# CPCLAB-UNIPI/MPC-code

Measured on AMD Instinct MI355X. Metric: closed-loop MPC steps/sec over batch, LMPC-CSTR N=50, higher is better.
Workload: dtype f64

## Files before the change

mpc-code_amd/csrc/mpc_wave.hpp:

```cpp
#pragma once
#include "mpc_device.hpp"
#include "mpc_tp.hpp"

namespace mpc {

#ifdef MPC_WV_GENERIC_TILES
constexpr bool kWvGenericTiles = true;
#else
constexpr bool kWvGenericTiles = false;
#endif

template <int NS, int NU, int NC, int NI_>
struct WvCfg {
    static constexpr int NI = NI_;
    static constexpr int NV = NS + NU, NKF = NU * NS, NLI = NU * (NU + 1) / 2;
    static constexpr int RA = 0, RA_SZ = (NC > NKF + NLI ? NC : NKF + NLI);
    static constexpr int RG = RA_SZ, RK = RG + NV, RZ = RK + NU, ROWS = RZ + 1;
    __host__ __device__ static constexpr int ld(int N) { return (N + 1) | 1; }
    static constexpr int GUARD = 8;
    __host__ __device__ static constexpr int t_doubles(int N) { return GUARD + ROWS * NI * ld(N); }
    static constexpr int RL_A = ROWS, RL_B = RL_A + NS * NS, RL_C = RL_B + NS * NU, ROWS_LTV = RL_C + NS;
    __host__ __device__ static constexpr int t_doubles_ltv(int N) { return GUARD + ROWS_LTV * NI * ld(N); }
    static constexpr int QZN = 5 * NS + 2 * NU + 1;
    static constexpr int QN = QZN + NS;
    static constexpr int ROWS_WS = NU + 2 * NC;
    static constexpr int OUT = NU + NS + 1;
    __host__ __device__ static constexpr size_t lds_doubles(int keep_per_inst, int N) { return (size_t)t_doubles(N) + NI * QN + NI * OUT + NI * keep_per_inst; }
};

template <int NS, int NU, int NC>
struct WvIter { double sl[NC], sh[NC], ll[NC], lh[NC], u[NU], z[NS]; };

struct AReg2 { int lo, hi; };
__device__ __forceinline__ void a_put(AReg2 &r, double v)
{
    union { double d; int i[2]; } u; u.d = v;
    asm("v_accvgpr_write_b32 %0, %1" : "=a"(r.lo) : "v"(u.i[0]));
    asm("v_accvgpr_write_b32 %0, %1" : "=a"(r.hi) : "v"(u.i[1]));
}
__device__ __forceinline__ double a_get(const AReg2 &r)
{
    union { double d; int i[2]; } u;
    asm("v_accvgpr_read_b32 %0, %1" : "=v"(u.i[0]) : "a"(r.lo));
    asm("v_accvgpr_read_b32 %0, %1" : "=v"(u.i[1]) : "a"(r.hi));
    return u.d;
}
template <int NS, int NU, int NC>
struct WvIterA {
    AReg2 sl[NC], sh[NC], ll[NC], lh[NC], u[NU], z[NS];
    __device__ __forceinline__ void get(WvIter<NS, NU, NC> &X) const
    {
        MPC_UNROLL for (int i = 0; i < NC; i++) { X.sl[i] = a_get(sl[i]); X.sh[i] = a_get(sh[i]); X.ll[i] = a_get(ll[i]); X.lh[i] = a_get(lh[i]); }
        MPC_UNROLL for (int i = 0; i < NU; i++) X.u[i] = a_get(u[i]);
        MPC_UNROLL for (int i = 0; i < NS; i++) X.z[i] = a_get(z[i]);
    }
    __device__ __forceinline__ void put(const WvIter<NS, NU, NC> &X)
    {
        MPC_UNROLL for (int i = 0; i < NC; i++) { a_put(sl[i], X.sl[i]); a_put(sh[i], X.sh[i]); a_put(ll[i], X.ll[i]); a_put(lh[i], X.lh[i]); }
        MPC_UNROLL for (int i = 0; i < NU; i++) a_put(u[i], X.u[i]);
        MPC_UNROLL for (int i = 0; i < NS; i++) a_put(z[i], X.z[i]);
    }
};

struct WvInst { double mu, mu_sum, sm, inv_ncon, gscale, res_s, res_p; int stall, iters, status; bool on, warm, keep_u; };

enum : int { kWvOk0 = 1, kWvWarm = 2, kWvValid = 4, kWvKeepU = 8, kWvNoShift = 16 };

__device__ __forceinline__ double row16_sum(double v)
{
    v += dpp_move<0xB1, 0xF>(0.0, v);
    v += dpp_move<0x4E, 0xF>(0.0, v);
    v += dpp_move<0x141, 0xF>(0.0, v);
    v += dpp_move<0x140, 0xF>(0.0, v);
    return v;
}
__device__ __forceinline__ double row16_max(double v)
{
    v = dmax(v, dpp_move<0xB1, 0xF>(v, v));
    v = dmax(v, dpp_move<0x4E, 0xF>(v, v));
    v = dmax(v, dpp_move<0x141, 0xF>(v, v));
    v = dmax(v, dpp_move<0x140, 0xF>(v, v));
    return v;
}

template <int NS, int NU, bool HASM, int NC, bool MASKED, int NI, class PT, bool LTV = false, bool PAIR = false, bool RES_P = false>
__device__ __forceinline__ void wv_solve(const PT &P, double *T, const double *q, const int *iflag,
                                         WvIterA<NS, NU, NC> (&X)[PAIR ? NI / 2 : NI], WvInst (&S)[PAIR ? NI / 2 : NI], int max_iter)
{
    static_assert(!LTV || (NS <= 4 && !HASM), "time-varying stage matrices: one 4 x 4 tile per state matrix, no cross term");
    using Cfg = WvCfg<NS, NU, NC, NI>;
    using Iter = WvIter<NS, NU, NC>;
    constexpr int NV = Cfg::NV, NKF = Cfg::NKF, NLI = Cfg::NLI, RA = Cfg::RA, RG = Cfg::RG, RK = Cfg::RK;
    static_assert(NS <= 8 && NU <= 2 && NI >= 1 && NI <= 4, "stage state <= 8 (2 x 2 tiles of 4 x 4), nu <= 2 (closed-form inverse of Lambda); at most four instances per product");
    static_assert(!PAIR || NI % 2 == 0, "pairs of instances");
    constexpr int NJ = PAIR ? NI / 2 : NI;
    const int lane = threadIdx.x, N = P.N, LD = Cfg::ld(N);
    const int k = PAIR ? (lane & 31) : lane;
    const int hsel = PAIR ? (lane >> 5) : 0;
    auto ji = [&](int j) -> int { return PAIR ? 2 * j + hsel : j; };
    const bool blk_on = k < N, last = k == N - 1;
    auto tk = [&](int row, int j) -> double & { return T[(row * NI + ji(j)) * LD + k]; };
    auto un = [](double v) -> double { return PAIR ? v : uni(v); };
    auto rsum = [](double v) -> double { return PAIR ? half_sum(v) : wave_sum(v); };
    auto rmax = [](double v) -> double { return PAIR ? half_max(v) : wave_max(v); };
    MPC_STAMP_INIT

    auto launder = [](const PT &Pin) -> const PT & { const PT *pp = &Pin; asm volatile("" : "+s"(pp)); return *pp; };
    struct Bnd { double lo[NC], hi[NC]; bool fl[NC], fh[NC]; };
    auto bounds = [&](const PT &Pl, int j, Bnd &Bd) {
        const double *qd = q + ji(j) * Cfg::QN;
        MPC_UNROLL for (int i = 0; i < NC; i++) {
// ... 137 lines not shown
                const bool f_lo = fin(ulo), f_hi = fin(uhi);
                double v;
                if (Sj.warm) {
                    const double t = wave_dn1(Xj.u[i], Xj.u[i]);
                    v = (rep || Sj.keep_u) ? Xj.u[i] : t;
                    if (f_lo) v = dmax(v, ulo);
                    if (f_hi) v = dmin(v, uhi);
                } else {
                    const double us = qd[5 * NS + NU + i];
                    double push;
                    if (f_lo && f_hi) push = 0.1 * (uhi - ulo);
                    else push = 0.1 * dmax(1.0, fabs(f_lo ? ulo : (f_hi ? uhi : 0.0)));
                    v = us;
                    if (f_lo) v = dmax(v, ulo + push);
                    if (f_hi) v = dmin(v, uhi - push);
                }
                Xj.u[i] = v;
            }
            MPC_UNROLL for (int i = 0; i < NC; i++) {
                if (Sj.warm) {
                    const double tl = wave_dn1(Xj.ll[i], Xj.ll[i]), th = wave_dn1(Xj.lh[i], Xj.lh[i]);
                    ll0[i] = rep ? Xj.ll[i] : tl; lh0[i] = rep ? Xj.lh[i] : th;
                } else { ll0[i] = 0.0; lh0[i] = 0.0; }
            }
            if (LTV) {
                double Ak[NS][NS], bk[NS], xk[NS];
                MPC_UNROLL for (int i = 0; i < NS; i++) {
                    double a = blk_on ? tk(Cfg::RL_C + i, j) : 0.0;
                    MPC_UNROLL for (int l = 0; l < NU; l++) a += (blk_on ? tk(Cfg::RL_B + i * NU + l, j) : 0.0) * Xj.u[l];
                    bk[i] = a;
                    MPC_UNROLL for (int l = 0; l < NS; l++) Ak[i][l] = blk_on ? tk(Cfg::RL_A + i * NS + l, j) : 0.0;
                }
                MPC_UNROLL for (int i = 0; i < NS; i++) { double a = bk[i]; MPC_UNROLL for (int l = 0; l < NS; l++) a += Ak[i][l] * qd[l]; xk[i] = k == 0 ? a : 0.0; }
                double x00[NS];
                MPC_UNROLL for (int i = 0; i < NS; i++) x00[i] = xk[i];
                if (k == 0 || !blk_on) { MPC_UNROLL for (int i = 0; i < NS; i++) { bk[i] = x00[i]; MPC_UNROLL for (int l = 0; l < NS; l++) Ak[i][l] = 0.0; } }
                for (int s = 1; s < N; s++) {
                    double t[NS];
                    MPC_UNROLL for (int i = 0; i < NS; i++) { const double v = wave_up1(xk[i], xk[i]); t[i] = (PAIR && (k == 0 || !blk_on)) ? 0.0 : v; }
                    MPC_UNROLL for (int i = 0; i < NS; i++) { double a = bk[i]; MPC_UNROLL for (int l = 0; l < NS; l++) a += Ak[i][l] * t[l]; xk[i] = a; }
                }
                MPC_UNROLL for (int i = 0; i < NS; i++) Xj.z[i] = xk[i];
            } else {
                double xk[NS];
                MPC_UNROLL for (int i = 0; i < NS; i++) {
                    double a = qd[2 * NS + i];
                    MPC_UNROLL for (int l = 0; l < NU; l++) a += Pl.B[i][l] * Xj.u[l];
                    if (k == 0) { MPC_UNROLL for (int l = 0; l < NS; l++) a += Pl.A[i][l] * qd[l]; }
                    xk[i] = blk_on ? a : 0.0;
                }
                MPC_UNROLL for (int e = 0; e < 6; e++) {
                    const int d = 1 << e;
                    if (d < N) {
                        double t[NS];
                        MPC_UNROLL for (int i = 0; i < NS; i++) { const double v = e == 0 ? wave_up1(xk[i], xk[i]) : __shfl_up(xk[i], d, 64); t[i] = k >= d ? v : 0.0; }
                        MPC_UNROLL for (int i = 0; i < NS; i++) { double a = xk[i]; MPC_UNROLL for (int l = 0; l < NS; l++) a += Pl.Apow[e][i][l] * t[l]; xk[i] = a; }
                    }
                }
                MPC_UNROLL for (int i = 0; i < NS; i++) Xj.z[i] = xk[i];
            }
            Bnd Bd; bounds(Pl, j, Bd);
            const double ws_delta = un(qd[5 * NS + 2 * NU]);
            const double ws_smin = dmin(dmax(kWsKappa * ws_delta, kWsSMinLo), kWsSMinHi), ws_mu = kWsMuFactor * ws_smin * ws_smin;
            const double smin = Sj.warm ? ws_smin : kSMin;
            MPC_UNROLL for (int i = 0; i < NC; i++) {
                const double v = i < NU ? Xj.u[i < NU ? i : 0] : Xj.z[i >= NU ? i - NU : 0];
                Xj.sl[i] = Bd.fl[i] ? dmax(v - Bd.lo[i], smin) : 1.0; Xj.sh[i] = Bd.fh[i] ? dmax(Bd.hi[i] - v, smin) : 1.0;
                const double isl = frcp(Xj.sl[i]), ish = frcp(Xj.sh[i]);
                const double llo = Sj.warm ? dmax(ll0[i], ws_mu * isl) : kMu0 * isl, lhi = Sj.warm ? dmax(lh0[i], ws_mu * ish) : kMu0 * ish;
                Xj.ll[i] = Bd.fl[i] ? llo : 0.0; Xj.lh[i] = Bd.fh[i] ? lhi : 0.0;
            }
            X[j].put(Xj);
            phase_a(Pl, j, Sj, Xj, 0);
        }
        __builtin_amdgcn_sched_barrier(0);
    }

    MPC_TSTAMP(1);
    auto mm = [](double a, double b, double c) { return __builtin_amdgcn_mfma_f64_4x4x4f64(a, b, c, 0, 0, 0); };
    constexpr int RZ = Cfg::RZ;
    constexpr int SB = (NS + 3) / 4;
    constexpr bool VF = SB == 1 && !HASM && !kWvGenericTiles;
#define MPC_MM "v_mfma_f64_4x4x4_4b_f64 "
    struct TileCtx {
        int tr, tc; bool live;
        double *Tt, *trash;
        double Ar[SB][SB], Atr[SB][SB], Br[SB], Btr[SB];
        double *p_hu, *p_hz[SB], *p_kf, *p_k[SB], *p_kt[SB], *p_li;
        const double *p_a, *p_at, *p_b, *p_bt;
    };
    auto tile_ctx = [&](const PT &Pl) {
        int lo = threadIdx.x;
        asm volatile("" : "+v"(lo));
        TileCtx c;
        c.tr = lo >> 4; c.tc = lo & 3;
        const int tbq = (lo >> 2) & 3;
        c.live = tbq < NI;
        const int tb = c.live ? tbq : 0;
        const int tr = c.tr, tc = c.tc;
        c.Tt = T + tb * LD; c.trash = T - Cfg::GUARD;
        auto trow = [&](int row) -> double * { return c.Tt + (c.live ? row : RZ) * (NI * LD); };
        MPC_UNROLL for (int i = 0; i < SB; i++) {
            const int ri = 4 * i + tr, ci = 4 * i + tc;
            MPC_UNROLL for (int j = 0; j < SB; j++) {
                const int cj = 4 * j + tc, rj = 4 * j + tr;
                c.Ar[i][j] = (ri < NS && cj < NS) ? Pl.A[ri < NS ? ri : 0][cj < NS ? cj : 0] : 0.0;
                c.Atr[i][j] = (ri < NS && cj < NS) ? Pl.A[cj < NS ? cj : 0][ri < NS ? ri : 0] : 0.0;
                (void)rj;
            }
            c.Br[i] = (ri < NS && tc < NU) ? Pl.B[ri < NS ? ri : 0][tc < NU ? tc : 0] : 0.0;
            c.Btr[i] = (tr < NU && ci < NS) ? Pl.B[ci < NS ? ci : 0][tr < NU ? tr : 0] : 0.0;
            c.p_hz[i] = trow(ri < NS ? RG + NU + ri : RZ);
            c.p_k[i] = trow((tr < NU && ci < NS) ? RA + tr * NS + ci : RZ);
            c.p_kt[i] = trow((ri < NS && tc < NU) ? RA + tc * NS + ri : RZ);
        }
        c.p_hu = trow(tr < NU ? RG + tr : RZ); c.p_kf = trow(tr < NU ? RK + tr : RZ);
        if (LTV) {
            c.p_a = trow((tr < NS && tc < NS) ? Cfg::RL_A + tr * NS + tc : RZ); c.p_at = trow((tr < NS && tc < NS) ? Cfg::RL_A + tc * NS + tr : RZ);
            c.p_b = trow((tr < NS && tc < NU) ? Cfg::RL_B + tr * NU + tc : RZ); c.p_bt = trow((tr < NU && tc < NS) ? Cfg::RL_B + tc * NU + tr : RZ);
        }
        const int li_i = tr > tc ? tr : tc, li_j = tr > tc ? tc : tr;
        c.p_li = trow((tr < NU && tc < NU) ? RA + NKF + li_i * (li_i + 1) / 2 + li_j : RZ);
        return c;
    };
    double pd_min = 1.0;
    constexpr int PD = SB == 1 ? 4 : 2;

    auto tile_factor = [&]() {
        const PT &Pl = launder(P);
        const TileCtx c = tile_ctx(Pl);
        const int tr = c.tr, tc = c.tc; const bool live = c.live;
        double *const trash = c.trash;
        auto trow = [&](int row) -> double * { return c.Tt + (live ? row : RZ) * (NI * LD); };
        const bool in_uu = tr < NU && tc < NU;
        const double Rr = in_uu ? Pl.R[tr][tc] : 0.0;
        double Qr[SB][SB], Mtr[SB], BE0[SB], BE1[SB];
        MPC_UNROLL for (int i = 0; i < SB; i++) {
            const int ri = 4 * i + tr, ci = 4 * i + tc;
            MPC_UNROLL for (int j = 0; j < SB; j++) { const int cj = 4 * j + tc; Qr[i][j] = (ri < NS && cj < NS) ? Pl.Q[ri < NS ? ri : 0][cj < NS ? cj : 0] : 0.0; }
            Mtr[i] = (HASM && tr < NU && ci < NS) ? Pl.M[ci < NS ? ci : 0][tr < NU ? tr : 0] : 0.0;
            BE0[i] = ri < NS ? Pl.B[ri < NS ? ri : 0][0] : 0.0; BE1[i] = (NU > 1 && ri < NS) ? Pl.B[ri < NS ? ri : 0][NU > 1 ? 1 : 0] : 0.0;
        }
        const double RE0 = tc < NU ? Pl.R[0][tc] : 0.0, RE1 = (NU > 1 && tc < NU) ? Pl.R[NU > 1 ? 1 : 0][tc] : 0.0;
        const double Ir = tr == tc ? 1.0 : 0.0;
        const double *q_sz[SB];
        MPC_UNROLL for (int i = 0; i < SB; i++) { const int ri = 4 * i + tr; q_sz[i] = trow((tr == tc && ri < NS && NU + ri < NC) ? RA + NU + ri : RZ) + (N - 1); }
        const double *q_su = trow((tr == tc && tr < NU) ? RA + tr : RZ) + (N - 1);
        const double *q_s0 = trow(tc == 0 ? RA : RZ) + (N - 1), *q_s1 = trow((NU > 1 && tc == 1) ? RA + 1 : RZ) + (N - 1);
        const double *q_hu = c.p_hu + (N - 1);
        const double *q_hz[SB];
        MPC_UNROLL for (int i = 0; i < SB; i++) q_hz[i] = c.p_hz[i] + (N - 1);
        const int ri2 = tr & 1;
        const double c_a = (NU > 1 && tc == 1 && ri2 == 1) ? -1.0 : 0.0, c_d = (NU > 1 && tc == 0 && ri2 == 0) ? -1.0 : 0.0;
        const double c_o = (NU > 1 && tc < 2 && ri2 != tc) ? 1.0 : 0.0, c_1 = (NU == 1 && tc == 0) ? -1.0 : 0.0;
        const double w_top = tr < NU ? 1.0 : 0.0;
        const double k_a = c_a * w_top, k_d = c_d * w_top, k_o = c_o * w_top, k_1 = c_1 * w_top;
        const bool st_l = tr >= 2 && tc < NU && tc <= tr - 2 && tr - 2 < NU, st_f3 = NS < 4 && tr < NU && tc == 3;
        double *q_st[SB]; int stp[SB];
        MPC_UNROLL for (int j = 0; j < SB; j++) {
            const int cj = 4 * j + tc;
            const bool st_k = tr < NU && cj < NS;
            const bool any = live && (st_k || (j == 0 && (st_l || st_f3)));
            q_st[j] = any ? trow(st_k ? RA + tr * NS + cj : (st_l ? RA + NKF + (tr - 2) * (tr - 1) / 2 + tc : RK + (tr < NU ? tr : 0))) + (N - 1) : trash + PD;
            stp[j] = any ? PD : 0;
        }
        const bool sel_k0 = tr < NU && tc < NS;
        const bool st_f = live && NS >= 4 && tr < NU && tc == 0;
        double *q_sf = st_f ? c.p_kf + (N - 1) : trash + PD;
        const int stpf = st_f ? PD : 0;
        double Pm[SB][SB], PC[SB];
        MPC_UNROLL for (int i = 0; i < SB; i++) {
            const int ri = 4 * i + tr;
            MPC_UNROLL for (int j = 0; j < SB; j++) { const int cj = 4 * j + tc; Pm[i][j] = (ri < NS && cj < NS) ? Pl.Pf[ri < NS ? ri : 0][cj < NS ? cj : 0] : 0.0; }
            PC[i] = 0.0;
        }
        constexpr int NF = 2 * SB + 4 + (LTV ? 3 : 0);
        double f[PD][NF];
        const double *q_a = LTV ? c.p_a + (N - 1) : nullptr, *q_b = LTV ? c.p_b + (N - 1) : nullptr, *q_bt = LTV ? c.p_bt + (N - 1) : nullptr;
        auto fetch = [&](int d, int off) {
            MPC_UNROLL for (int i = 0; i < SB; i++) { f[d][i] = q_sz[i][off]; f[d][SB + 4 + i] = q_hz[i][off]; }
            f[d][SB] = q_su[off]; f[d][SB + 1] = q_s0[off]; f[d][SB + 2] = NU > 1 ? q_s1[off] : 0.0; f[d][SB + 3] = q_hu[off];
            if (LTV) { f[d][NF - 3] = q_a[off]; f[d][NF - 2] = q_b[off]; f[d][NF - 1] = q_bt[off]; }
        };
        MPC_UNROLL for (int d = 0; d < PD; d++) fetch(d, -d);
        auto block = [&](int d, bool more) {
            double sz[SB], HZ[SB];
            MPC_UNROLL for (int i = 0; i < SB; i++) { sz[i] = f[d][i]; HZ[i] = f[d][SB + 4 + i]; }
            const double su = f[d][SB], s0 = f[d][SB + 1], s1 = f[d][SB + 2], HU = f[d][SB + 3];
            double Arl[SB][SB], Brl[SB], Btrl[SB], BE0l[SB], BE1l[SB];
            MPC_UNROLL for (int i = 0; i < SB; i++) { Brl[i] = c.Br[i]; Btrl[i] = c.Btr[i]; BE0l[i] = BE0[i]; BE1l[i] = BE1[i]; MPC_UNROLL for (int jj = 0; jj < SB; jj++) Arl[i][jj] = c.Ar[i][jj]; }
            if (LTV) {
                Arl[0][0] = f[d][NF - 3]; Brl[0] = f[d][NF - 2]; Btrl[0] = f[d][NF - 1];
                BE0l[0] = dpp_move<0x00, 0xF>(Brl[0], Brl[0]); BE1l[0] = NU > 1 ? dpp_move<0x55, 0xF>(Brl[0], Brl[0]) : 0.0;
            }
            if (more) fetch(d, -PD - d);
            MPC_UNROLL for (int i = 0; i < SB; i++) Pm[i][i] += sz[i];
            if constexpr (VF) {
                const double X0i = RE0 + s0, X1i = RE1 + s1, PV0 = HZ[0] + PC[0], Rs = Rr + su;
                double PB, BtP, PA, psv, X0, X1, Psi;
                asm("s_nop 1\n\t"
                    MPC_MM "%0, %7, %8, 0\n\t"
                    MPC_MM "%1, %8, %7, 0\n\t"
                    MPC_MM "%2, %7, %9, 0\n\t"
                    MPC_MM "%3, %8, %10, %11\n\t"
                    "s_nop 2\n\t"
                    MPC_MM "%4, %12, %0, %14\n\t"
                    MPC_MM "%5, %13, %0, %15\n\t"
                    MPC_MM "%6, %8, %2, 0\n\t"
                    "s_nop 5"
                    : "=&v"(PB), "=&v"(BtP), "=&v"(PA), "=&v"(psv), "=&v"(X0), "=&v"(X1), "=&v"(Psi)
                    : "v"(Pm[0][0]), "v"(Brl[0]), "v"(Arl[0][0]), "v"(PV0), "v"(HU), "v"(BE0l[0]), "v"(BE1l[0]), "v"(X0i), "v"(X1i));
                const double a = dpp_move<0x00, 0xF>(X0, X0);
                double adjm, adjk, det;
                if (NU == 1) { det = a; adjm = c_1; adjk = k_1; pd_min = dmin(pd_min, a); }
                else {
                    const double off = dpp_move<0x55, 0xF>(X0, X0), dd = dpp_move<0x55, 0xF>(X1, X1);
                    det = __builtin_fma(a, dd, -(off * off));
                    adjk = __builtin_fma(k_d, dd, __builtin_fma(k_a, a, k_o * off));
                    adjm = __builtin_fma(c_d, dd, __builtin_fma(c_a, a, c_o * off));
                    pd_min = dmin(pd_min, dmin(a, det));
                }
                double Kk0;
                asm("s_nop 1\n\t" MPC_MM "%0, %2, %3, 0" : "=v"(Kk0), "+v"(det) : "v"(adjk), "v"(Psi));
                const double rdet = frcp(det);
                asm("s_nop 1" : "+v"(Kk0) : "v"(rdet));
                Kk0 *= rdet;
                const double mL = adjm * rdet, mLi = adjk * rdet;
                double RK0, Acl0, Tm0, a2, KFF, acc, acc2, PCn;
                asm("s_nop 1\n\t"
                    MPC_MM "%0, %8, %9, 0\n\t"
                    MPC_MM "%1, %10, %9, %11\n\t"
                    MPC_MM "%2, %12, %9, %13\n\t"
                    MPC_MM "%3, %9, %14, 0\n\t"
                    MPC_MM "%4, %15, %16, 0\n\t"
                    "s_nop 2\n\t"
                    MPC_MM "%5, %9, %0, %17\n\t"
                    MPC_MM "%6, %1, %2, 0\n\t"
                    MPC_MM "%7, %1, %18, %3\n\t"
                    "s_nop 5"
                    : "=&v"(RK0), "=&v"(Acl0), "=&v"(Tm0), "=&v"(a2), "=&v"(KFF), "=&v"(acc), "=&v"(acc2), "=&v"(PCn)
                    : "v"(Rs), "v"(Kk0), "v"(Btrl[0]), "v"(Arl[0][0]), "v"(BtP), "v"(PA), "v"(HU), "v"(mLi), "v"(psv), "v"(Qr[0][0]), "v"(PV0));
                q_st[0][-d] = sel_k0 ? Kk0 : (st_l ? mL : KFF);
                if (NS >= 4) q_sf[-d] = KFF;
                Pm[0][0] = acc + acc2;
                PC[0] = PCn;
                return;
            }
            double PA[SB][SB], PB[SB], BtP[SB];
            MPC_UNROLL for (int i = 0; i < SB; i++) {
                double pb = 0.0, bp = 0.0;
                MPC_UNROLL for (int l = 0; l < SB; l++) { pb = mm(Pm[l][i], Brl[l], pb); bp = mm(Brl[l], Pm[l][i], bp); }
                PB[i] = pb; BtP[i] = bp;
                MPC_UNROLL for (int j = 0; j < SB; j++) { double a = 0.0; MPC_UNROLL for (int l = 0; l < SB; l++) a = mm(Pm[l][i], Arl[l][j], a); PA[i][j] = a; }
            }
            double X0 = RE0 + s0, X1 = RE1 + s1;
            MPC_UNROLL for (int l = 0; l < SB; l++) { X0 = mm(BE0l[l], PB[l], X0); if (NU > 1) X1 = mm(BE1l[l], PB[l], X1); }
            double Psi[SB];
            MPC_UNROLL for (int j = 0; j < SB; j++) { double a = Mtr[j]; MPC_UNROLL for (int l = 0; l < SB; l++) a = mm(Brl[l], PA[l][j], a); Psi[j] = a; }
            const double Rs = Rr + su;
            const double a = dpp_move<0x00, 0xF>(X0, X0);
            double adjm, adjk, det;
            if (NU == 1) { det = a; adjm = c_1; adjk = k_1; pd_min = dmin(pd_min, a); }
            else {
                const double off = dpp_move<0x55, 0xF>(X0, X0), dd = dpp_move<0x55, 0xF>(X1, X1);
                det = __builtin_fma(a, dd, -(off * off));
                adjk = __builtin_fma(k_d, dd, __builtin_fma(k_a, a, k_o * off));
                adjm = __builtin_fma(c_d, dd, __builtin_fma(c_a, a, c_o * off));
                pd_min = dmin(pd_min, dmin(a, det));
            }
            double Kk[SB];
            MPC_UNROLL for (int j = 0; j < SB; j++) Kk[j] = mm(adjk, Psi[j], 0.0);
            const double rdet = frcp(det);
            MPC_UNROLL for (int j = 0; j < SB; j++) Kk[j] *= rdet;
            const double mL = adjm * rdet, mLi = adjk * rdet;
            double PV[SB], psv = HU;
            MPC_UNROLL for (int i = 0; i < SB; i++) { PV[i] = HZ[i] + PC[i]; psv = mm(Brl[i], PV[i], psv); }
            const double KFF = mm(mLi, psv, 0.0);
            q_st[0][-d] = sel_k0 ? Kk[0] : (st_l ? mL : KFF);
            MPC_UNROLL for (int j = 1; j < SB; j++) q_st[j][-d] = Kk[j];
            if (NS >= 4) q_sf[-d] = KFF;
            double Acl[SB][SB], Tm[SB][SB], RK_[SB], MK[SB][SB];
            MPC_UNROLL for (int j = 0; j < SB; j++) RK_[j] = mm(Rs, Kk[j], 0.0);
            MPC_UNROLL for (int i = 0; i < SB; i++) {
                MPC_UNROLL for (int j = 0; j < SB; j++) {
                    Acl[i][j] = mm(Btrl[i], Kk[j], Arl[i][j]);
                    Tm[i][j] = mm(BtP[i], Kk[j], PA[i][j]);
                    if (HASM) MK[i][j] = mm(Mtr[i], Kk[j], 0.0);
                }
            }
            MPC_UNROLL for (int i = 0; i < SB; i++) {
                MPC_UNROLL for (int j = 0; j < SB; j++) {
                    double acc = mm(Kk[i], RK_[j], Qr[i][j]), acc2 = 0.0;
                    MPC_UNROLL for (int l = 0; l < SB; l++) acc2 = mm(Acl[l][i], Tm[l][j], acc2);
                    double pn = acc + acc2;
                    if (HASM) pn = mm(MK[j][i], Ir, pn + MK[i][j]);
                    Pm[i][j] = pn;
                }
            }
            MPC_UNROLL for (int i = 0; i < SB; i++) { double a2 = mm(Kk[i], HU, 0.0); MPC_UNROLL for (int l = 0; l < SB; l++) a2 = mm(Acl[l][i], PV[l], a2); PC[i] = a2; }
        };
        const int G = N / PD, rem = N - G * PD;
        for (int g = 0; g < G; g++) {
            MPC_UNROLL for (int d = 0; d < PD; d++) block(d, true);
            MPC_UNROLL for (int i = 0; i < SB; i++) { q_sz[i] -= PD; q_hz[i] -= PD; q_st[i] -= stp[i]; }
            q_su -= PD; q_s0 -= PD; q_s1 -= PD; q_hu -= PD; q_sf -= stpf;
            if (LTV) { q_a -= PD; q_b -= PD; q_bt -= PD; }
        }
        MPC_UNROLL for (int d = 0; d < PD - 1; d++) { if (d < rem) block(d, false); }
    };
    auto tile_rhs = [&]() {
        const PT &Pl = launder(P);
        const TileCtx c = tile_ctx(Pl);
        const int tr = c.tr, tc = c.tc; const bool live = c.live;
        double *const trash = c.trash;
        const bool st_any = live && tr < NU && tc == 0;
        const double *q_hu = c.p_hu + (N - 1), *q_li = c.p_li + (N - 1);
        const double *q_hz[SB], *q_k[SB];
        MPC_UNROLL for (int i = 0; i < SB; i++) { q_hz[i] = c.p_hz[i] + (N - 1); q_k[i] = c.p_k[i] + (N - 1); }
        double *q_st = st_any ? c.p_kf + (N - 1) : trash + PD;
        const int stp = st_any ? PD : 0;
        double PC[SB];
        MPC_UNROLL for (int i = 0; i < SB; i++) PC[i] = 0.0;
        constexpr int NF = 2 * SB + 2 + (LTV ? 3 : 0);
        double f[PD][NF];
        const double *q_a = LTV ? c.p_a + (N - 1) : nullptr, *q_b = LTV ? c.p_b + (N - 1) : nullptr, *q_bt = LTV ? c.p_bt + (N - 1) : nullptr;
        auto fetch = [&](int d, int off) {
            f[d][0] = q_hu[off]; f[d][1] = q_li[off];
            MPC_UNROLL for (int i = 0; i < SB; i++) { f[d][2 + i] = q_hz[i][off]; f[d][2 + SB + i] = q_k[i][off]; }
            if (LTV) { f[d][NF - 3] = q_a[off]; f[d][NF - 2] = q_b[off]; f[d][NF - 1] = q_bt[off]; }
        };
        MPC_UNROLL for (int d = 0; d < PD; d++) fetch(d, -d);
        auto block = [&](int d, bool more) {
            const double HU = f[d][0], mLi = f[d][1];
            double HZ[SB], Kk[SB];
            MPC_UNROLL for (int i = 0; i < SB; i++) { HZ[i] = f[d][2 + i]; Kk[i] = f[d][2 + SB + i]; }
            double Arl[SB][SB], Brl[SB], Btrl[SB];
            MPC_UNROLL for (int i = 0; i < SB; i++) { Brl[i] = c.Br[i]; Btrl[i] = c.Btr[i]; MPC_UNROLL for (int jj = 0; jj < SB; jj++) Arl[i][jj] = c.Ar[i][jj]; }
            if (LTV) { Arl[0][0] = f[d][NF - 3]; Brl[0] = f[d][NF - 2]; Btrl[0] = f[d][NF - 1]; }
            if (more) fetch(d, -PD - d);
            if constexpr (VF) {
                const double PV0 = HZ[0] + PC[0];
                double Acl0, psv, cst0, KFF, cst, dyn;
                asm("s_nop 1\n\t"
                    MPC_MM "%0, %6, %7, %8\n\t"
                    MPC_MM "%1, %9, %10, %11\n\t"
                    MPC_MM "%2, %7, %11, 0\n\t"
                    "s_nop 4\n\t"
                    MPC_MM "%3, %12, %1, 0\n\t"
                    MPC_MM "%4, %0, %13, %2\n\t"
                    MPC_MM "%5, %0, %14, 0\n\t"
                    "s_nop 6"
                    : "=&v"(Acl0), "=&v"(psv), "=&v"(cst0), "=&v"(KFF), "=&v"(cst), "=&v"(dyn)
                    : "v"(Btrl[0]), "v"(Kk[0]), "v"(Arl[0][0]), "v"(Brl[0]), "v"(PV0), "v"(HU), "v"(mLi), "v"(HZ[0]), "v"(PC[0]));
                q_st[-d] = KFF;
                PC[0] = cst + dyn;
                return;
            }
            double psv = HU;
            MPC_UNROLL for (int i = 0; i < SB; i++) psv = mm(Brl[i], HZ[i] + PC[i], psv);
            q_st[-d] = mm(mLi, psv, 0.0);
            double Acl[SB][SB], PCn[SB];
            MPC_UNROLL for (int i = 0; i < SB; i++) { MPC_UNROLL for (int j = 0; j < SB; j++) Acl[i][j] = mm(Btrl[i], Kk[j], Arl[i][j]); }
            MPC_UNROLL for (int i = 0; i < SB; i++) {
                double cst = mm(Kk[i], HU, 0.0), dyn = 0.0;
                MPC_UNROLL for (int l = 0; l < SB; l++) { cst = mm(Acl[l][i], HZ[l], cst); dyn = mm(Acl[l][i], PC[l], dyn); }
                PCn[i] = cst + dyn;
            }
            MPC_UNROLL for (int i = 0; i < SB; i++) PC[i] = PCn[i];
        };
        const int G = N / PD, rem = N - G * PD;
        for (int g = 0; g < G; g++) {
            MPC_UNROLL for (int d = 0; d < PD; d++) block(d, true);
            MPC_UNROLL for (int i = 0; i < SB; i++) { q_hz[i] -= PD; q_k[i] -= PD; }
            q_hu -= PD; q_li -= PD; q_st -= stp;
            if (LTV) { q_a -= PD; q_b -= PD; q_bt -= PD; }
        }
        MPC_UNROLL for (int d = 0; d < PD - 1; d++) { if (d < rem) block(d, false); }
    };
    auto tile_forward = [&]() {
        const PT &Pl = launder(P);
        const TileCtx c = tile_ctx(Pl);
        const int tr = c.tr, tc = c.tc; const bool live = c.live;
        double *const trash = c.trash;
        auto trow = [&](int row) -> double * { return c.Tt + (live ? row : RZ) * (NI * LD); };
        const bool st_u = tr < NU && tc == 0;
        double *q_st[SB]; int stp[SB];
        MPC_UNROLL for (int i = 0; i < SB; i++) {
            const int ri = 4 * i + tr;
            const bool st_z = ri < NS && tc == 1;
            const bool any = live && (st_z || (i == 0 && st_u));
            q_st[i] = any ? trow((i == 0 && st_u) ? RG + tr : RG + NU + (ri < NS ? ri : 0)) : trash;
            stp[i] = any ? PD : 0;
        }
        const double *q_kf = c.p_kf;
        const double *q_k[SB], *q_kt[SB];
        MPC_UNROLL for (int i = 0; i < SB; i++) { q_k[i] = c.p_k[i]; q_kt[i] = c.p_kt[i]; }
        double DZ[SB];
        MPC_UNROLL for (int i = 0; i < SB; i++) DZ[i] = 0.0;
        constexpr int NF = 2 * SB + 1 + (LTV ? 2 : 0);
        double f[PD][NF];
        const double *q_at = LTV ? c.p_at : nullptr, *q_bt = LTV ? c.p_bt : nullptr;
        auto fetch = [&](int d, int off) {
            f[d][0] = q_kf[off];
            MPC_UNROLL for (int i = 0; i < SB; i++) { f[d][1 + i] = q_k[i][off]; f[d][1 + SB + i] = q_kt[i][off]; }
            if (LTV) { f[d][NF - 2] = q_at[off]; f[d][NF - 1] = q_bt[off]; }
        };
        MPC_UNROLL for (int d = 0; d < PD; d++) fetch(d, d);
        auto block = [&](int d, bool more) {
            const double KFF = f[d][0];
            double Kk[SB], KkT[SB];
            MPC_UNROLL for (int i = 0; i < SB; i++) { Kk[i] = f[d][1 + i]; KkT[i] = f[d][1 + SB + i]; }
            double Atrl[SB][SB], Btrl[SB];
            MPC_UNROLL for (int i = 0; i < SB; i++) { Btrl[i] = c.Btr[i]; MPC_UNROLL for (int jj = 0; jj < SB; jj++) Atrl[i][jj] = c.Atr[i][jj]; }
            if (LTV) { Atrl[0][0] = f[d][NF - 2]; Btrl[0] = f[d][NF - 1]; }
            if (more) fetch(d, PD + d);
            if constexpr (VF) {
                double Aclt, a0, DUv, DZn0;
                asm("s_nop 1\n\t"
                    MPC_MM "%0, %4, %5, %6\n\t"
                    MPC_MM "%1, %5, %7, 0\n\t"
                    MPC_MM "%2, %8, %9, %7\n\t"
                    "s_nop 3\n\t"
                    MPC_MM "%3, %0, %9, %1\n\t"
                    "s_nop 5"
                    : "=&v"(Aclt), "=&v"(a0), "=&v"(DUv), "=&v"(DZn0)
                    : "v"(Kk[0]), "v"(Btrl[0]), "v"(Atrl[0][0]), "v"(KFF), "v"(KkT[0]), "v"(DZ[0]));
                q_st[0][d] = st_u ? DUv : DZn0;
                DZ[0] = DZn0;
                return;
            }
            double DU = KFF;
            MPC_UNROLL for (int j = 0; j < SB; j++) DU = mm(KkT[j], DZ[j], DU);
            double DZn[SB];
            MPC_UNROLL for (int i = 0; i < SB; i++) {
                double a = mm(Btrl[i], KFF, 0.0);
                MPC_UNROLL for (int j = 0; j < SB; j++) a = mm(mm(Kk[j], Btrl[i], Atrl[j][i]), DZ[j], a);
                DZn[i] = a;
            }
            q_st[0][d] = st_u ? DU : DZn[0];
            MPC_UNROLL for (int i = 1; i < SB; i++) q_st[i][d] = DZn[i];
            MPC_UNROLL for (int i = 0; i < SB; i++) DZ[i] = DZn[i];
        };
        const int G = N / PD, rem = N - G * PD;
        for (int g = 0; g < G; g++) {
            MPC_UNROLL for (int d = 0; d < PD; d++) block(d, true);
            MPC_UNROLL for (int i = 0; i < SB; i++) { q_k[i] += PD; q_kt[i] += PD; q_st[i] += stp[i]; }
            q_kf += PD;
            if (LTV) { q_at += PD; q_bt += PD; }
        }
        MPC_UNROLL for (int d = 0; d < PD - 1; d++) { if (d < rem) block(d, false); }
    };

    AReg2 dvp[NJ][NC];
    for (int it = 0;; it++) {
        bool any_on = false;
        MPC_UNROLL for (int j = 0; j < NJ; j++) any_on = any_on || (PAIR ? __any(S[j].on) != 0 : S[j].on);
        if (!any_on) break;
        __syncthreads();
        pd_min = 1.0;
        tile_factor();
        __syncthreads();
        MPC_TSTAMP(2);
        tile_forward();
        __syncthreads();
        MPC_TSTAMP(3);
        {
            const unsigned long long bad = __ballot(((lane >> 2) & 3) < NI && !(pd_min > 0.0));
            MPC_UNROLL for (int j = 0; j < NJ; j++) {
                if (S[j].on && (bad & (0x000F000F000F000FULL << (4 * ji(j))))) { S[j].on = false; S[j].status = kInfeasible; S[j].iters = it; }
            }
        }
        MPC_UNROLL for (int j = 0; j < NJ; j++) {
            WvInst &Sj = S[j];
            if (Sj.on) {
                Iter Xj; X[j].get(Xj);
                const PT &Pl = P;
                Bnd Bd; bounds(Pl, j, Bd);
                double maff_p = 1.0, s1_p = 0.0, s2_p = 0.0, pl[NC], ph[NC], dvj[NC];
                MPC_UNROLL for (int i = 0; i < NC; i++) { dvj[i] = tk(RG + i, j); a_put(dvp[j][i], dvj[i]); }
                MPC_UNROLL for (int i = 0; i < NC; i++) {
                    const double v = i < NU ? Xj.u[i < NU ? i : 0] : Xj.z[i >= NU ? i - NU : 0];
                    const double isl = frcp(Xj.sl[i]), ish = frcp(Xj.sh[i]);
                    const double rh = Bd.fh[i] ? v + Xj.sh[i] - Bd.hi[i] : 0.0, rl = Bd.fl[i] ? v - Xj.sl[i] - Bd.lo[i] : 0.0;
                    const double dsh = Bd.fh[i] ? -rh - dvj[i] : 0.0, dsl = Bd.fl[i] ? rl + dvj[i] : 0.0;
                    const double qh = dsh * ish, ql = dsl * isl;
                    const double dlh = Bd.fh[i] ? -Xj.lh[i] - Xj.lh[i] * qh : 0.0, dll = Bd.fl[i] ? -Xj.ll[i] - Xj.ll[i] * ql : 0.0;
                    maff_p = dmax(maff_p, dmax(-ql, -qh));
                    if (Bd.fl[i]) maff_p = dmax(maff_p, 1.0 + ql);
                    if (Bd.fh[i]) maff_p = dmax(maff_p, 1.0 + qh);
                    s1_p += Xj.sl[i] * dll + Xj.ll[i] * dsl + Xj.sh[i] * dlh + Xj.lh[i] * dsh;
                    s2_p += dsl * dll + dsh * dlh;
                    pl[i] = dsl * dll; ph[i] = dsh * dlh;
                }
                const double m_aff = rmax(blk_on ? maff_p : 1.0), s1 = rsum(blk_on ? s1_p : 0.0), s2 = rsum(blk_on ? s2_p : 0.0);
                const double a_aff = frcp(m_aff);
                const double mu_aff = (Sj.mu_sum + a_aff * s1 + a_aff * a_aff * s2) * Sj.inv_ncon;
                const double rat = Sj.mu > 0.0 ? mu_aff * frcp(Sj.mu) : 0.0;
                Sj.sm = dmax(rat * rat * rat * Sj.mu, kMuFloor);
                double gu[NU], gz[NS], hc[NV];
                gradient(Pl, j, Xj, gu, gz);
                MPC_UNROLL for (int i = NC; i < NV; i++) hc[i] = 0.0;
                MPC_UNROLL for (int i = 0; i < NC; i++) {
                    const double v = i < NU ? Xj.u[i < NU ? i : 0] : Xj.z[i >= NU ? i - NU : 0];
                    const double isl = frcp(Xj.sl[i]), ish = frcp(Xj.sh[i]);
                    const double rh = Bd.fh[i] ? v + Xj.sh[i] - Bd.hi[i] : 0.0, rl = Bd.fl[i] ? v - Xj.sl[i] - Bd.lo[i] : 0.0;
                    const double rch = Bd.fh[i] ? Xj.sh[i] * Xj.lh[i] - dmax(Sj.sm, Xj.lh[i] * kSFloor) + ph[i] : 0.0;
                    const double rcl = Bd.fl[i] ? Xj.sl[i] * Xj.ll[i] - dmax(Sj.sm, Xj.ll[i] * kSFloor) + pl[i] : 0.0;
                    hc[i] = (-rch + Xj.lh[i] * rh) * ish + (rcl + Xj.ll[i] * rl) * isl;
                }
                if (blk_on) {
                    MPC_UNROLL for (int i = 0; i < NU; i++) tk(RG + i, j) = gu[i] + hc[i];
                    MPC_UNROLL for (int i = 0; i < NS; i++) tk(RG + NU + i, j) = gz[i] + hc[NU + i];
                }
            }
            __builtin_amdgcn_sched_barrier(0);
        }
        __syncthreads();
        MPC_TSTAMP(4);
        tile_rhs();
        __syncthreads();
        MPC_TSTAMP(5);
        tile_forward();
        __syncthreads();
        MPC_TSTAMP(3);
        MPC_UNROLL for (int j = 0; j < NJ; j++) {
            WvInst &Sj = S[j];
            if (Sj.on) {
                Iter Xj; X[j].get(Xj);
                const PT &Pl = P;
                Bnd Bd; bounds(Pl, j, Bd);
                double dvzj[NV], dvj[NC];
                MPC_UNROLL for (int i = 0; i < NC; i++) dvj[i] = a_get(dvp[j][i]);
                MPC_UNROLL for (int i = 0; i < NV; i++) dvzj[i] = tk(RG + i, j);
                double mcc_p = kTau;
                double dsl[NC], dsh[NC], dll[NC], dlh[NC];
                MPC_UNROLL for (int i = 0; i < NC; i++) {
                    const double v = i < NU ? Xj.u[i < NU ? i : 0] : Xj.z[i >= NU ? i - NU : 0];
                    const double isl = frcp(Xj.sl[i]), ish = frcp(Xj.sh[i]);
                    const double rh = Bd.fh[i] ? v + Xj.sh[i] - Bd.hi[i] : 0.0, rl = Bd.fl[i] ? v - Xj.sl[i] - Bd.lo[i] : 0.0;
                    const double ash = Bd.fh[i] ? -rh - dvj[i] : 0.0, asl = Bd.fl[i] ? rl + dvj[i] : 0.0;
                    const double alh = Bd.fh[i] ? -Xj.lh[i] - Xj.lh[i] * (ash * ish) : 0.0, all_ = Bd.fl[i] ? -Xj.ll[i] - Xj.ll[i] * (asl * isl) : 0.0;
                    const double rch = Bd.fh[i] ? Xj.sh[i] * Xj.lh[i] - dmax(Sj.sm, Xj.lh[i] * kSFloor) + ash * alh : 0.0;
                    const double rcl = Bd.fl[i] ? Xj.sl[i] * Xj.ll[i] - dmax(Sj.sm, Xj.ll[i] * kSFloor) + asl * all_ : 0.0;
                    dsh[i] = Bd.fh[i] ? -rh - dvzj[i] : 0.0; dsl[i] = Bd.fl[i] ? rl + dvzj[i] : 0.0;
                    dlh[i] = Bd.fh[i] ? (-rch - Xj.lh[i] * dsh[i]) * ish : 0.0; dll[i] = Bd.fl[i] ? (-rcl - Xj.ll[i] * dsl[i]) * isl : 0.0;
                    mcc_p = dmax(mcc_p, dmax(-dsl[i] * isl, -dsh[i] * ish));
                    if (Bd.fl[i]) mcc_p = dmax(mcc_p, -dll[i] * frcp_approx(Xj.ll[i]));
                    if (Bd.fh[i]) mcc_p = dmax(mcc_p, -dlh[i] * frcp_approx(Xj.lh[i]));
                }
                const double m_cc = rmax(blk_on ? mcc_p : kTau);
                const double alpha = m_cc <= kTau ? 1.0 : kTau * frcp(m_cc);
                MPC_UNROLL for (int i = 0; i < NC; i++) { Xj.sl[i] += alpha * dsl[i]; Xj.sh[i] += alpha * dsh[i]; Xj.ll[i] += alpha * dll[i]; Xj.lh[i] += alpha * dlh[i]; }
                MPC_UNROLL for (int i = 0; i < NU; i++) Xj.u[i] += alpha * dvzj[i];
                MPC_UNROLL for (int i = 0; i < NS; i++) Xj.z[i] += alpha * dvzj[NU + i];
                X[j].put(Xj);
                phase_a(Pl, j, Sj, Xj, it + 1);
            }
            __builtin_amdgcn_sched_barrier(0);
        }
        MPC_TSTAMP(6);
    }
}
#undef MPC_MM



template <int NX, int NU, int NY, int ND, int NGS = 0, int NHS = 0>
struct Row16Tab {
    static constexpr int NE = NX + ND, NR = NU - NHS, NCT = NX + NU + NY + NGS;
    static constexpr int E_A = 0, E_Q = NE, E_K = 2 * NE, E_DMIN = 2 * NE + NY, E_DMAX = E_DMIN + 1, ESZ = E_DMAX + 1;
    static constexpr int T_W = 0, T_LO = NR, T_HI = NR + 1, TSZ = NR + 2;
    static constexpr int DOUBLES = NE * ESZ + NCT * TSZ;
#ifdef MPC_ROW16_OFF
    static constexpr bool fits = false;
#else
    static constexpr bool fits = NE <= 16 && NCT <= 16;
#endif
    static constexpr int XCH = NE * NY + NE * NE;
};

template <int NX, int NU, int NY, int ND, int NGS = 0, int NHS = 0, class PT>
__device__ __forceinline__ void row16_fill_tables(const PT &P, double *tab, int lane)
{
    using RT = Row16Tab<NX, NU, NY, ND, NGS, NHS>;
    constexpr int NE = RT::NE;
    if (lane < NE) {
        double *e = tab + lane * RT::ESZ;
        for (int j = 0; j < NE; j++) { e[RT::E_A + j] = P.Aa[lane][j]; e[RT::E_Q + j] = P.Qkf[lane][j]; }
        for (int j = 0; j < NY; j++) e[RT::E_K + j] = P.Kfix[lane][j];
        e[RT::E_DMIN] = lane >= NX ? P.dmin[lane - NX] : 0.0; e[RT::E_DMAX] = lane >= NX ? P.dmax[lane - NX] : 0.0;
    }
    if (lane < RT::NCT) {
        double *t = tab + NE * RT::ESZ + lane * RT::TSZ;
        constexpr int NVY = NX + NU + NY;
        if (NGS == 0 || lane < NVY) {
            for (int c = 0; c < RT::NR; c++) t[RT::T_W + c] = P.W[lane][c];
            t[RT::T_LO] = P.tlo[lane]; t[RT::T_HI] = P.thi[lane];
        } else if constexpr (NGS > 0) {
            for (int c = 0; c < RT::NR; c++) t[RT::T_W + c] = P.Wg[lane - NVY][c];
            t[RT::T_LO] = -INFINITY; t[RT::T_HI] = 0.0;
        }
    }
}

template <int NX, int NY, int ND, int NXP, int NU, class PT>
__device__ __forceinline__ void kalman_row16(const PT &P, int r, bool slot_on, double *kp, int x_off, int xi_off, int p_off, const double *pyp_k,
                                             const double *vn_k, size_t Bs, const double *tab, double *xch, double &xi_old, double &xi_new)
{
    using RT = Row16Tab<NX, NU, NY, ND>;
    constexpr int NE = RT::NE;
    const bool row = r < NE && slot_on;
    const int rr = r < NE ? r : 0;
    const double *e = tab + rr * RT::ESZ;
    double xi[NE], innov[NY];
    MPC_UNROLL for (int i = 0; i < NE; i++) xi[i] = kp[xi_off + i];
    MPC_UNROLL for (int i = 0; i < NY; i++) {
        double yh = P.fyc[i], yy = pyp_k[i];
        if (vn_k) yy += vn_k[i * Bs];
        MPC_UNROLL for (int j = 0; j < NE; j++) yh += P.Ca[i][j] * xi[j];
        MPC_UNROLL for (int j = 0; j < NXP; j++) yy += P.Cp[i][j] * kp[x_off + j];
        innov[i] = yy - yh;
    }
    xi_old = kp[xi_off + rr];
    double Kr[NY];
    if (P.estimator == MPC_EST_KALMAN) {
        double Pr[NE], PCt[NY];
        MPC_UNROLL for (int j = 0; j < NE; j++) Pr[j] = kp[p_off + rr * NE + j];
        MPC_UNROLL for (int j = 0; j < NY; j++) { double a = 0.0; MPC_UNROLL for (int l = 0; l < NE; l++) a += Pr[l] * P.Ca[j][l]; PCt[j] = a; }
        if (row) { MPC_UNROLL for (int j = 0; j < NY; j++) xch[r * NY + j] = PCt[j]; }
        __syncthreads();
        double all[NE][NY], S[NY][NY];
        MPC_UNROLL for (int l = 0; l < NE; l++) { MPC_UNROLL for (int j = 0; j < NY; j++) all[l][j] = xch[l * NY + j]; }
        MPC_UNROLL for (int i = 0; i < NY; i++) { MPC_UNROLL for (int j = 0; j < NY; j++) { double a = P.Rkf[i][j]; MPC_UNROLL for (int l = 0; l < NE; l++) a += P.Ca[i][l] * all[l][j]; S[i][j] = a; } }
        MPC_UNROLL for (int i = 0; i < NY; i++) { MPC_UNROLL for (int j = 0; j < i; j++) { const double a = 0.5 * (S[i][j] + S[j][i]); S[i][j] = a; S[j][i] = a; } }
        sym_inverse<NY>(S);
        MPC_UNROLL for (int j = 0; j < NY; j++) { double a = 0.0; MPC_UNROLL for (int l = 0; l < NY; l++) a += PCt[l] * S[l][j]; Kr[j] = a; }
        double Pc[NE], U[NE];
        MPC_UNROLL for (int j = 0; j < NE; j++) { double a = Pr[j]; MPC_UNROLL for (int m = 0; m < NY; m++) a -= Kr[m] * all[j][m]; Pc[j] = a; }
        MPC_UNROLL for (int j = 0; j < NE; j++) { double a = 0.0; MPC_UNROLL for (int l = 0; l < NE; l++) a += Pc[l] * P.Aa[j][l]; U[j] = a; }
        double *xu = xch + NE * NY;
        if (row) { MPC_UNROLL for (int j = 0; j < NE; j++) xu[r * NE + j] = U[j]; }
        __syncthreads();
        double Pn[NE];
        MPC_UNROLL for (int j = 0; j < NE; j++) Pn[j] = e[RT::E_Q + j];
        MPC_UNROLL for (int l = 0; l < NE; l++) { const double al = e[RT::E_A + l]; MPC_UNROLL for (int j = 0; j < NE; j++) Pn[j] += al * xu[l * NE + j]; }
        if (row) { MPC_UNROLL for (int j = 0; j < NE; j++) kp[p_off + r * NE + j] = Pn[j]; }
// ... 158 lines not shown
```

Measured before the change: 34.12 million.

## Interleave LDS prefetch reads into MFMA asm blocks for factor, rhs and forward sweeps

For the scalar-state, time-invariant case, the three Riccati-style sweeps (factorisation, backward rhs, forward substitution) get hand-written inline-asm steps. Each step issues the ds_read_b64 prefetches for a later stage inside the same asm block as the MFMA chain, with explicit lgkmcnt waits and a compile-time unrolled ring of four stages. The goal is to hide LDS latency behind the dependent MFMA chain and remove compiler-inserted waits and scheduling gaps. The cost is brittle hand-scheduled assembly with manual nop and waitcnt hazards, which could give wrong results or stalls if a timing assumption is off.

```diff
diff --git a/mpc-code_amd/csrc/mpc_wave.hpp b/mpc-code_amd/csrc/mpc_wave.hpp
--- a/mpc-code_amd/csrc/mpc_wave.hpp
+++ b/mpc-code_amd/csrc/mpc_wave.hpp
@@ -27,6 +27,9 @@
     static constexpr int OUT = NU + NS + 1;
     __host__ __device__ static constexpr size_t lds_doubles(int keep_per_inst, int N) { return (size_t)t_doubles(N) + NI * QN + NI * OUT + NI * keep_per_inst; }
 };
+
+template <int V>
+struct WvInt { static constexpr int value = V; };
 
 template <int NS, int NU, int NC>
 struct WvIter { double sl[NC], sh[NC], ll[NC], lh[NC], u[NU], z[NS]; };
@@ -330,6 +333,9 @@
     constexpr int SB = (NS + 3) / 4;
     constexpr bool VF = SB == 1 && !HASM && !kWvGenericTiles;
 #define MPC_MM "v_mfma_f64_4x4x4_4b_f64 "
+#define MPC_WV_RD(dst, addr) "ds_read_b64 %[" #dst "], %[" #addr "] offset:%[off]\n\t"
+#define MPC_WV_NORD(dst, addr) "s_nop 0\n\t"
+    auto wv_lds_addr = [](const double *p) { return (unsigned)(unsigned long long)p; };
     struct TileCtx {
         int tr, tc; bool live;
         double *Tt, *trash;
@@ -431,6 +437,92 @@
             if (LTV) { f[d][NF - 3] = q_a[off]; f[d][NF - 2] = q_b[off]; f[d][NF - 1] = q_bt[off]; }
         };
         MPC_UNROLL for (int d = 0; d < PD; d++) fetch(d, -d);
+        if constexpr (VF && !LTV) {
+            unsigned a_sz = wv_lds_addr(q_sz[0]) - 64, a_su = wv_lds_addr(q_su) - 64, a_s0 = wv_lds_addr(q_s0) - 64, a_s1 = wv_lds_addr(q_s1) - 64;
+            unsigned a_hu = wv_lds_addr(q_hu) - 64, a_hz = wv_lds_addr(q_hz[0]) - 64;
+            const double Br0 = c.Br[0], Btr0 = c.Btr[0], Ar0 = c.Ar[0][0], BE00 = BE0[0], BE10 = BE1[0], Qr0 = Qr[0][0];
+            double Pm0 = Pm[0][0], PC0 = 0.0;
+            auto step = [&](auto D, auto MORE) {
+                constexpr int d = decltype(D)::value, dp = (d + PD - 1) % PD;
+                constexpr bool more = decltype(MORE)::value;
+                Pm0 += f[d][0];
+                const double X0i = RE0 + f[d][2], X1i = RE1 + f[d][3], PV0 = f[d][5] + PC0, Rs = Rr + f[d][1];
+                double PB, BtP, PA, psv, X0, X1, Psi;
+#define MPC_FAC_STMT1(RD) \
+                "s_nop 1\n\t" \
+                MPC_MM "%[pb], %[pm], %[br], 0\n\t" \
+                MPC_MM "%[btp], %[br], %[pm], 0\n\t" \
+                MPC_MM "%[pa], %[pm], %[ar], 0\n\t" \
+                MPC_MM "%[psv], %[br], %[pv], %[hu]\n\t" \
+                RD(sz, asz) RD(su, asu) RD(s0, as0) \
+                MPC_MM "%[x0], %[be0], %[pb], %[x0i]\n\t" \
+                MPC_MM "%[x1], %[be1], %[pb], %[x1i]\n\t" \
+                RD(s1, as1) \
+                MPC_MM "%[psi], %[br], %[pa], 0\n\t" \
+                RD(hz, ahz) \
+                "s_nop 4" \
+                : [pb] "=&v"(PB), [btp] "=&v"(BtP), [pa] "=&v"(PA), [psv] "=&v"(psv), [x0] "=&v"(X0), [x1] "=&v"(X1), [psi] "=&v"(Psi), \
+                  [sz] "+v"(f[d][0]), [su] "+v"(f[d][1]), [s0] "+v"(f[d][2]), [s1] "+v"(f[d][3]), [hz] "+v"(f[d][5]) \
+                : [pm] "v"(Pm0), [br] "v"(Br0), [ar] "v"(Ar0), [pv] "v"(PV0), [hu] "v"(f[d][4]), [be0] "v"(BE00), [be1] "v"(BE10), [x0i] "v"(X0i), [x1i] "v"(X1i), \
+                  [asz] "v"(a_sz), [asu] "v"(a_su), [as0] "v"(a_s0), [as1] "v"(a_s1), [ahz] "v"(a_hz), [off] "i"((PD - d) * 8) : "memory"
+                if constexpr (more) asm volatile(MPC_FAC_STMT1(MPC_WV_RD));
+                else asm volatile(MPC_FAC_STMT1(MPC_WV_NORD));
+#undef MPC_FAC_STMT1
+                const double a = dpp_move<0x00, 0xF>(X0, X0);
+                double adjm, adjk, det;
+                if (NU == 1) { det = a; adjm = c_1; adjk = k_1; pd_min = dmin(pd_min, a); }
+                else {
+                    const double off = dpp_move<0x55, 0xF>(X0, X0), dd = dpp_move<0x55, 0xF>(X1, X1);
+                    det = __builtin_fma(a, dd, -(off * off));
+                    adjk = __builtin_fma(k_d, dd, __builtin_fma(k_a, a, k_o * off));
+                    adjm = __builtin_fma(c_d, dd, __builtin_fma(c_a, a, c_o * off));
+                    pd_min = dmin(pd_min, dmin(a, det));
+                }
+                double Kk0;
+                asm volatile("s_waitcnt lgkmcnt(0)\n\ts_nop 0\n\t" MPC_MM "%[kk], %[adjk], %[psi], 0"
+                             : [kk] "=v"(Kk0), "+v"(det), "+v"(f[d][0]), "+v"(f[d][1]), "+v"(f[d][2]), "+v"(f[d][3]), "+v"(f[d][5]), "+v"(f[dp][4])
+                             : [adjk] "v"(adjk), [psi] "v"(Psi) : "memory");
+                const double rdet = frcp(det);
+                asm("s_nop 1" : "+v"(Kk0) : "v"(rdet));
+                Kk0 *= rdet;
+                const double mL = adjm * rdet, mLi = adjk * rdet;
+                double RK0, Acl0, Tm0, a2, KFF, acc, acc2, PCn;
+#define MPC_FAC_STMT3(RD) \
+                "s_nop 1\n\t" \
+                MPC_MM "%[rk], %[rs], %[kk], 0\n\t" \
+                MPC_MM "%[acl], %[btr], %[kk], %[ar]\n\t" \
+                MPC_MM "%[tm], %[btp], %[kk], %[pa]\n\t" \
+                MPC_MM "%[a2], %[kk], %[hu], 0\n\t" \
+                RD(hu, ahu) \
+                MPC_MM "%[kff], %[mli], %[psv], 0\n\t" \
+                "s_nop 1\n\t" \
+                MPC_MM "%[acc], %[kk], %[rk], %[q]\n\t" \
+                MPC_MM "%[acc2], %[acl], %[tm], 0\n\t" \
+                MPC_MM "%[pcn], %[acl], %[pv], %[a2]\n\t" \
+                "s_nop 5" \
+                : [rk] "=&v"(RK0), [acl] "=&v"(Acl0), [tm] "=&v"(Tm0), [a2] "=&v"(a2), [kff] "=&v"(KFF), [acc] "=&v"(acc), [acc2] "=&v"(acc2), [pcn] "=&v"(PCn), [hu] "+v"(f[d][4]) \
+                : [rs] "v"(Rs), [kk] "v"(Kk0), [btr] "v"(Btr0), [ar] "v"(Ar0), [btp] "v"(BtP), [pa] "v"(PA), [mli] "v"(mLi), [psv] "v"(psv), [q] "v"(Qr0), [pv] "v"(PV0), \
+                  [ahu] "v"(a_hu), [off] "i"((PD - d) * 8) : "memory"
+                if constexpr (more) asm volatile(MPC_FAC_STMT3(MPC_WV_RD));
+                else asm volatile(MPC_FAC_STMT3(MPC_WV_NORD));
+#undef MPC_FAC_STMT3
+                q_st[0][-d] = sel_k0 ? Kk0 : (st_l ? mL : KFF);
+                if (NS >= 4) q_sf[-d] = KFF;
+                Pm0 = acc + acc2;
+                PC0 = PCn;
+            };
+            const int G = N / PD, rem = N - G * PD;
+            for (int g = 0; g < G; g++) {
+                step(WvInt<0>{}, WvInt<1>{}); step(WvInt<1>{}, WvInt<1>{}); step(WvInt<2>{}, WvInt<1>{}); step(WvInt<3>{}, WvInt<1>{});
+                a_sz -= PD * 8; a_su -= PD * 8; a_s0 -= PD * 8; a_s1 -= PD * 8; a_hu -= PD * 8; a_hz -= PD * 8;
+                q_st[0] -= stp[0]; q_sf -= stpf;
+            }
+            if (0 < rem) step(WvInt<0>{}, WvInt<0>{});
+            if (1 < rem) step(WvInt<1>{}, WvInt<0>{});
+            if (2 < rem) step(WvInt<2>{}, WvInt<0>{});
+            asm volatile("s_waitcnt lgkmcnt(0)" : "+v"(f[0][4]), "+v"(f[1][4]), "+v"(f[2][4]), "+v"(f[3][4]));
+            return;
+        }
         auto block = [&](int d, bool more) {
             double sz[SB], HZ[SB];
             MPC_UNROLL for (int i = 0; i < SB; i++) { sz[i] = f[d][i]; HZ[i] = f[d][SB + 4 + i]; }
@@ -578,6 +670,63 @@
             if (LTV) { f[d][NF - 3] = q_a[off]; f[d][NF - 2] = q_b[off]; f[d][NF - 1] = q_bt[off]; }
         };
         MPC_UNROLL for (int d = 0; d < PD; d++) fetch(d, -d);
+        if constexpr (VF && !LTV) {
+            unsigned a_hu = wv_lds_addr(q_hu) - 64, a_li = wv_lds_addr(q_li) - 64, a_hz = wv_lds_addr(q_hz[0]) - 64, a_k = wv_lds_addr(q_k[0]) - 64;
+            const double Br0 = c.Br[0], Btr0 = c.Btr[0], Ar0 = c.Ar[0][0];
+            double PC0 = 0.0, Acl0, cstc;
+            {
+                double cst0;
+                asm volatile("s_nop 1\n\t"
+                             MPC_MM "%0, %3, %4, %5\n\t"
+                             MPC_MM "%1, %4, %6, 0\n\t"
+                             "s_nop 4\n\t"
+                             MPC_MM "%2, %0, %7, %1\n\t"
+                             "s_nop 1"
+                             : "=&v"(Acl0), "=&v"(cst0), "=&v"(cstc) : "v"(Btr0), "v"(f[0][3]), "v"(Ar0), "v"(f[0][0]), "v"(f[0][2]));
+            }
+#define MPC_RHS_STMT(RD, W) \
+            "s_nop 1\n\t" \
+            MPC_MM "%[dyn], %[acl], %[pc], 0\n\t" \
+            MPC_MM "%[psv], %[br], %[pv], %[hu]\n\t" \
+            RD(hu, ahu) \
+            MPC_MM "%[acln], %[btr], %[k1], %[ar]\n\t" \
+            RD(hz, ahz) \
+            MPC_MM "%[cst0n], %[k1], %[hu1], 0\n\t" \
+            RD(k, ak) \
+            "s_nop 0\n\t" \
+            MPC_MM "%[kff], %[li], %[psv], 0\n\t" \
+            RD(li, ali) \
+            MPC_MM "%[cstn], %[acln], %[hz1], %[cst0n]\n\t" \
+            "s_waitcnt lgkmcnt(" W ")\n\t" \
+            "s_nop 5" \
+            : [dyn] "=&v"(dyn), [psv] "=&v"(psv), [acln] "=&v"(AclN), [cst0n] "=&v"(cst0N), [kff] "=&v"(KFF), [cstn] "=&v"(cstN), \
+              [hu] "+v"(f[d][0]), [li] "+v"(f[d][1]), [hz] "+v"(f[d][2]), [k] "+v"(f[d][3]), "+v"(f[dp][0]), "+v"(f[dp][1]), "+v"(f[dp][2]), "+v"(f[dp][3]) \
+            : [acl] "v"(Acl0), [pc] "v"(PC0), [pv] "v"(PV0), [br] "v"(Br0), [btr] "v"(Btr0), [ar] "v"(Ar0), [hu1] "v"(f[dn][0]), [hz1] "v"(f[dn][2]), [k1] "v"(f[dn][3]), \
+              [ahu] "v"(a_hu), [ali] "v"(a_li), [ahz] "v"(a_hz), [ak] "v"(a_k), [off] "i"((PD - d) * 8) : "memory"
+            auto step = [&](auto D, auto MORE) {
+                constexpr int d = decltype(D)::value, dn = (d + 1) % PD, dp = (d + PD - 1) % PD;
+                const double PV0 = f[d][2] + PC0;
+                double dyn, psv, AclN, cst0N, KFF, cstN;
+                if constexpr (decltype(MORE)::value) asm volatile(MPC_RHS_STMT(MPC_WV_RD, "4"));
+                else asm volatile(MPC_RHS_STMT(MPC_WV_NORD, "0"));
+                q_st[-d] = KFF;
+                PC0 = cstc + dyn;
+                cstc = cstN; Acl0 = AclN;
+            };
+#undef MPC_RHS_STMT
+            const int G = N / PD, rem = N - G * PD;
+            for (int g = 0; g < G; g++) {
+                step(WvInt<0>{}, WvInt<1>{}); step(WvInt<1>{}, WvInt<1>{}); step(WvInt<2>{}, WvInt<1>{}); step(WvInt<3>{}, WvInt<1>{});
+                a_hu -= PD * 8; a_li -= PD * 8; a_hz -= PD * 8; a_k -= PD * 8; q_st -= stp;
+            }
+            if (0 < rem) step(WvInt<0>{}, WvInt<0>{});
+            if (1 < rem) step(WvInt<1>{}, WvInt<0>{});
+            if (2 < rem) step(WvInt<2>{}, WvInt<0>{});
+            asm volatile("s_waitcnt lgkmcnt(0)"
+                         : "+v"(f[0][0]), "+v"(f[0][1]), "+v"(f[0][2]), "+v"(f[0][3]), "+v"(f[1][0]), "+v"(f[1][1]), "+v"(f[1][2]), "+v"(f[1][3]),
+                           "+v"(f[2][0]), "+v"(f[2][1]), "+v"(f[2][2]), "+v"(f[2][3]), "+v"(f[3][0]), "+v"(f[3][1]), "+v"(f[3][2]), "+v"(f[3][3]), "+v"(Acl0), "+v"(cstc));
+            return;
+        }
         auto block = [&](int d, bool more) {
             const double HU = f[d][0], mLi = f[d][1];
             double HZ[SB], Kk[SB];
@@ -654,6 +803,52 @@
             if (LTV) { f[d][NF - 2] = q_at[off]; f[d][NF - 1] = q_bt[off]; }
         };
         MPC_UNROLL for (int d = 0; d < PD; d++) fetch(d, d);
+        if constexpr (VF && !LTV) {
+            unsigned a_kf = wv_lds_addr(q_kf), a_k = wv_lds_addr(q_k[0]), a_kt = wv_lds_addr(q_kt[0]);
+            const double Btr0 = c.Btr[0], Atr0 = c.Atr[0][0];
+            double DZ0 = 0.0, Aclt, a0;
+            asm volatile("s_nop 1\n\t"
+                         MPC_MM "%0, %2, %3, %4\n\t"
+                         MPC_MM "%1, %3, %5, 0\n\t"
+                         "s_nop 2"
+                         : "=&v"(Aclt), "=&v"(a0) : "v"(f[0][1]), "v"(Btr0), "v"(Atr0), "v"(f[0][0]));
+#define MPC_FWD_STMT(RD, W) \
+            "s_nop 1\n\t" \
+            MPC_MM "%[dzn], %[aclt], %[dz], %[a0]\n\t" \
+            RD(k, ak) \
+            MPC_MM "%[du], %[kt], %[dz], %[kf]\n\t" \
+            RD(kf, akf) \
+            RD(kt, akt) \
+            MPC_MM "%[acltn], %[k1], %[btr], %[atr]\n\t" \
+            MPC_MM "%[a0n], %[btr], %[kf1], 0\n\t" \
+            "s_waitcnt lgkmcnt(" W ")\n\t" \
+            "s_nop 1" \
+            : [dzn] "=&v"(DZn), [du] "=&v"(DUv), [acltn] "=&v"(AcltN), [a0n] "=&v"(a0N), [kf] "+v"(f[d][0]), [k] "+v"(f[d][1]), [kt] "+v"(f[d][2]), \
+              "+v"(f[dp][0]), "+v"(f[dp][1]), "+v"(f[dp][2]) \
+            : [aclt] "v"(Aclt), [a0] "v"(a0), [dz] "v"(DZ0), [kf1] "v"(f[dn][0]), [k1] "v"(f[dn][1]), [btr] "v"(Btr0), [atr] "v"(Atr0), \
+              [akf] "v"(a_kf), [ak] "v"(a_k), [akt] "v"(a_kt), [off] "i"((PD + d) * 8) : "memory"
+            auto step = [&](auto D, auto MORE) {
+                constexpr int d = decltype(D)::value, dn = (d + 1) % PD, dp = (d + PD - 1) % PD;
+                double DZn, DUv, AcltN, a0N;
+                if constexpr (decltype(MORE)::value) asm volatile(MPC_FWD_STMT(MPC_WV_RD, "3"));
+                else asm volatile(MPC_FWD_STMT(MPC_WV_NORD, "0"));
+                q_st[0][d] = st_u ? DUv : DZn;
+                DZ0 = DZn; Aclt = AcltN; a0 = a0N;
+            };
+#undef MPC_FWD_STMT
+            const int G = N / PD, rem = N - G * PD;
+            for (int g = 0; g < G; g++) {
+                step(WvInt<0>{}, WvInt<1>{}); step(WvInt<1>{}, WvInt<1>{}); step(WvInt<2>{}, WvInt<1>{}); step(WvInt<3>{}, WvInt<1>{});
+                a_kf += PD * 8; a_k += PD * 8; a_kt += PD * 8; q_st[0] += stp[0];
+            }
+            if (0 < rem) step(WvInt<0>{}, WvInt<0>{});
+            if (1 < rem) step(WvInt<1>{}, WvInt<0>{});
+            if (2 < rem) step(WvInt<2>{}, WvInt<0>{});
+            asm volatile("s_waitcnt lgkmcnt(0)\n\ts_nop 5"
+                         : "+v"(f[0][0]), "+v"(f[0][1]), "+v"(f[0][2]), "+v"(f[1][0]), "+v"(f[1][1]), "+v"(f[1][2]), "+v"(f[2][0]), "+v"(f[2][1]), "+v"(f[2][2]),
+                           "+v"(f[3][0]), "+v"(f[3][1]), "+v"(f[3][2]), "+v"(Aclt), "+v"(a0));
+            return;
+        }
         auto block = [&](int d, bool more) {
             const double KFF = f[d][0];
             double Kk[SB], KkT[SB];
@@ -810,6 +1005,8 @@
     }
 }
 #undef MPC_MM
+#undef MPC_WV_RD
+#undef MPC_WV_NORD
 
 
 
```

Measured after the change: 35.86 million (median of 6 runs). +5.1%, better.
